# JackShDr/InfluentialRS

Measured on AMD Instinct MI355X. Metric: scored user-item pairs/sec (whole node), higher is better.
Workload: dtype f32; 1 GPU; c2: n_item=3415, d=128, L=200, H=4, layers=6, ffn=256; one greedy path-search step; users_per_gpu=4096, top_k=100, sweep=bf16 filter + exact f32 re-score, parallelism=single GPU

## Files before the change

### influentialrs_amd/csrc/capi.hip

```cpp
#include <stdlib.h>

#include <new>

#include "irs_internal.h"

int irs_launch_topk_exhaustive(irs_ctx *ctx, const float *xrows, int M, int k, float *val, int64_t *ids0,
                               int32_t *status, hipStream_t s);

static char g_create_err[512] = "";

static inline size_t align_up(size_t v, size_t a) { return (v + a - 1) / a * a; }

extern "C" int irs_abi_version(void) { return IRS_ABI_VERSION; }

extern "C" const char *irs_last_error(const irs_ctx *ctx) { return ctx ? ctx->err : g_create_err; }

extern "C" int irs_create(irs_ctx **out, const irs_dims *dims, const irs_shard *shard) {
    if (!out || !dims) {
        snprintf(g_create_err, sizeof(g_create_err), "irs_create: null argument");
        return IRS_E_INVALID;
    }
    const irs_dims &D = *dims;
#define BAD(...)                                                   \
    do {                                                           \
        snprintf(g_create_err, sizeof(g_create_err), __VA_ARGS__); \
        return IRS_E_INVALID;                                      \
    } while (0)
    if (D.n_item < 1) BAD("n_item must be >= 1");
    if (D.d < 2 || D.d > 256 || (D.d & 1)) BAD("emb_dim must be even and in [2, 256] (got %d)", D.d);
    if (D.max_len < 2 || D.max_len > 256) BAD("max_len must be in [2, 256] (got %d)", D.max_len);
    if (D.n_heads < 1 || D.d % D.n_heads) BAD("n_heads must divide emb_dim");
    if (D.d / D.n_heads > 64) BAD("head dim > 64 unsupported");
    if (D.n_layers < 1 || D.n_layers > IRS_MAX_LAYERS) BAD("n_layers out of range");
    if (D.ffn_dim < 1) BAD("ffn_dim must be >= 1");
    if (D.mask_mode != IRS_MASK_IRN && D.mask_mode != IRS_MASK_CAUSAL) BAD("bad mask_mode");
    if (D.mask_mode == IRS_MASK_IRN && (D.u_dim < 1 || D.n_user < 1)) BAD("IRN mask needs user embeddings");
    if (D.max_rows < 1) BAD("max_rows must be >= 1");
    if (D.max_k < 1 || D.max_k > 1024) BAD("max_k must be in [1, 1024]");
    irs_shard sh;
    if (shard) sh = *shard;
    else {
        sh.rank = 0;
        sh.world = 1;
        sh.item_lo = 0;
        sh.item_hi = D.n_item;
    }
    if (sh.item_lo < 0 || sh.item_hi > D.n_item || sh.item_lo >= sh.item_hi) BAD("bad item shard [%lld, %lld)", (long long)sh.item_lo, (long long)sh.item_hi);
    if (sh.item_hi - sh.item_lo > 0x7FFFFFE0LL) BAD("shard too large");
    {
        int dev = 0;
        if (hipGetDevice(&dev) == hipSuccess && (dev < 0 || dev >= IRS_MAX_DEVICES))
            BAD("device ordinal %d: contexts are supported on devices 0 .. %d", dev, IRS_MAX_DEVICES - 1);
    }
#undef BAD
    irs_ctx *c = new (std::nothrow) irs_ctx();
    if (!c) {
        snprintf(g_create_err, sizeof(g_create_err), "out of host memory");
        return IRS_E_INVALID;
    }
    memset(c, 0, sizeof(*c));
    c->dims = D;
    c->shard = sh;
    c->n_local = sh.item_hi - sh.item_lo;
    int dp = 16;
    while (dp < D.d) dp <<= 1;
    c->d_pad = dp;
    c->KS = dp / 16;
    c->n_tiles = (int)((c->n_local + 31) / 32);
    c->max_rows = D.max_rows;
    c->max_seqs = D.max_seqs > 0 ? D.max_seqs : D.max_rows;
    c->m_pad_max = (c->max_rows + 31) & ~31;
    c->lse_slots = 2048;
    {
        const char *e = getenv("IRS_DECODER_GEMM");
        if (e && strcmp(e, "f32") && strcmp(e, "x6") && strcmp(e, "h3")) {
            snprintf(g_create_err, sizeof(g_create_err), "IRS_DECODER_GEMM=%s (expected h3, x6 or f32)", e);
            delete c;
            return IRS_E_INVALID;
        }
        c->use_x6 = e ? (strcmp(e, "f32") == 0 ? IRS_GEMM_F32 : strcmp(e, "x6") == 0 ? IRS_GEMM_X6 : IRS_GEMM_H3) : IRS_GEMM_H3;
        const char *ea = getenv("IRS_ATTN_GEMM");
        if (ea && strcmp(ea, "f32") && strcmp(ea, "h3")) {
            snprintf(g_create_err, sizeof(g_create_err), "IRS_ATTN_GEMM=%s (expected h3 or f32)", ea);
            delete c;
            return IRS_E_INVALID;
        }
        c->use_attn_h3 = ea ? (strcmp(ea, "h3") == 0) : 1;
        const char *es = getenv("IRS_DECODER_SEQ");
        c->use_seq = es ? (strcmp(es, "auto") == 0 ? 2 : (atoi(es) != 0 ? 1 : 0)) : 2;
        const char *ec = getenv("IRS_THR_CARRY");
        c->carry_period = ec ? atoi(ec) : 8;
        if (c->carry_period < 0 || c->carry_period > 1024) c->carry_period = 8;
        const char *eo = getenv("IRS_SHARDED_OVERLAP");
        c->sh_overlap = eo ? (atoi(eo) != 0 ? 1 : 0) : 0;
        const char *er = getenv("IRS_LSE_RING");
        c->lse_no_ring = er ? (strcmp(er, "0") == 0) : 0;
    }
    *out = c;
    return IRS_OK;
}

extern "C" void irs_destroy(irs_ctx *ctx) {
    if (!ctx) return;
    if (ctx->graph_exec) hipGraphExecDestroy(ctx->graph_exec);
    if (ctx->beam_graph) hipGraphExecDestroy(ctx->beam_graph);
    if (ctx->sh_graph) hipGraphExecDestroy(ctx->sh_graph);
    if (ctx->sh_side) {
        for (int i = 0; i < 8; ++i) (void)hipEventDestroy(ctx->sh_ev[i]);
        (void)hipStreamDestroy(ctx->sh_side);
    }
    if (ctx->prof_ev) {
        for (int i = 0; i < ctx->prof_cap; ++i) {
            hipEventDestroy(ctx->prof_ev[i].a);
            hipEventDestroy(ctx->prof_ev[i].b);
        }
        free(ctx->prof_ev);
    }
    delete ctx;
}

static bool ends_with(const char *s, const char *suf) {
    size_t ls = strlen(s), lf = strlen(suf);
    return ls >= lf && strcmp(s + ls - lf, suf) == 0;
}

extern "C" int irs_bind_weight(irs_ctx *ctx, const char *name, const float *p, int64_t numel) {
    if (!ctx || !name || !p) return IRS_E_INVALID;
    if (strncmp(name, "module.", 7) == 0) name += 7;
    const irs_dims &D = ctx->dims;
    const int64_t d = D.d, F = D.ffn_dim;
    const float **slot = nullptr;
    int64_t want = -1;
    if (!strcmp(name, "item_embedder.weight") || !strcmp(name, "word_embedder.weight")) {
        slot = &ctx->item_emb;
        want = (D.n_item + 1) * d;
    } else if (!strcmp(name, "user_embedder.weight")) {
        slot = &ctx->user_emb;
        want = D.n_user * D.u_dim;
    } else if (!strcmp(name, "pos_embedder.pe")) {
        slot = &ctx->pe;
        want = -2;
        if (numel < (int64_t)D.max_len * d) IRS_FAIL(ctx, IRS_E_INVALID, "pos_embedder.pe too small");
    } else if (!strcmp(name, "user_mask_layer.weight")) {
        slot = &ctx->um_w;
        want = D.u_dim;
    } else if (!strcmp(name, "user_mask_layer.bias")) {
        slot = &ctx->um_b;
        want = 1;
    } else if (!strcmp(name, "project.weight")) {
        slot = &ctx->proj_w;
        want = ctx->n_local * d;
    } else if (!strcmp(name, "project.bias")) {
        slot = &ctx->proj_b;
        want = ctx->n_local;
    } else if (!strncmp(name, "decoder.layers.", 15)) {
        char *end = nullptr;
        long l = strtol(name + 15, &end, 10);
        if (l < 0 || l >= D.n_layers || !end || *end != '.') IRS_FAIL(ctx, IRS_E_INVALID, "bad layer in '%s'", name);
        const char *rest = end + 1;
        irs_layer_w &w = ctx->layer[l];
        struct { const char *n; const float **s; int64_t numel; } tab[] = {
            {"self_attn.in_proj_weight", &w.sa_in_w, 3 * d * d}, {"self_attn.in_proj_bias", &w.sa_in_b, 3 * d},
            {"self_attn.out_proj.weight", &w.sa_out_w, d * d},   {"self_attn.out_proj.bias", &w.sa_out_b, d},
            {"multihead_attn.in_proj_weight", &w.ca_in_w, 3 * d * d}, {"multihead_attn.in_proj_bias", &w.ca_in_b, 3 * d},
            {"multihead_attn.out_proj.weight", &w.ca_out_w, d * d},   {"multihead_attn.out_proj.bias", &w.ca_out_b, d},
            {"linear1.weight", &w.l1_w, F * d}, {"linear1.bias", &w.l1_b, F},
            {"linear2.weight", &w.l2_w, d * F}, {"linear2.bias", &w.l2_b, d},
            {"norm1.weight", &w.n1_w, d}, {"norm1.bias", &w.n1_b, d},
            {"norm2.weight", &w.n2_w, d}, {"norm2.bias", &w.n2_b, d},
            {"norm3.weight", &w.n3_w, d}, {"norm3.bias", &w.n3_b, d},
        };
        for (auto &e : tab)
            if (!strcmp(rest, e.n)) {
                slot = e.s;
                want = e.numel;
            }
    }
    if (!slot) IRS_FAIL(ctx, IRS_E_INVALID, "unknown weight '%s'", name);
    if (want >= 0 && numel != want) IRS_FAIL(ctx, IRS_E_INVALID, "weight '%s': numel %lld, expected %lld", name, (long long)numel, (long long)want);
    *slot = p;
    ctx->finalized = false;
    (void)ends_with;
    return IRS_OK;
}

static int check_bound(irs_ctx *ctx) {
    const irs_dims &D = ctx->dims;
    if (!ctx->item_emb || !ctx->pe || !ctx->proj_w || !ctx->proj_b) IRS_FAIL(ctx, IRS_E_STATE, "embedding / pe / project weights not bound");
    if (D.mask_mode == IRS_MASK_IRN && (!ctx->user_emb || !ctx->um_w || !ctx->um_b)) IRS_FAIL(ctx, IRS_E_STATE, "user weights not bound");
    for (int l = 0; l < D.n_layers; ++l) {
        const irs_layer_w &w = ctx->layer[l];
        const float *all[] = {w.sa_in_w, w.sa_in_b, w.sa_out_w, w.sa_out_b, w.ca_in_b, w.ca_out_w, w.ca_out_b, w.l1_w,
                              w.l1_b, w.l2_w, w.l2_b, w.n1_w, w.n1_b, w.n2_w, w.n2_b, w.n3_w, w.n3_b};
        for (auto p : all)
            if (!p) IRS_FAIL(ctx, IRS_E_STATE, "decoder layer %d has unbound weights", l);
    }
    return IRS_OK;
}

static size_t derived_plan(const irs_ctx *ctx, size_t *o_wp, size_t *o_bias, size_t *o_cl, size_t *o_wn, size_t *o_wf, size_t *o_x6 = nullptr) {
    size_t off = 0;
    *o_wp = off;
    off = align_up(off + (size_t)ctx->n_tiles * ctx->KS * 1024, 256);
    *o_bias = off;
    off = align_up(off + (size_t)ctx->n_tiles * 32 * sizeof(float), 256);
    *o_cl = off;
    off = align_up(off + (size_t)ctx->dims.n_layers * ctx->dims.d * sizeof(float), 256);
    *o_wn = off;
    off = align_up(off + 256, 256);
    *o_wf = off;
    off = align_up(off + irs_small_frag_floats(ctx) * sizeof(float), 256);
    if (o_x6) *o_x6 = off;
    off = align_up(off + irs_x6_bytes(ctx), 256);
    return off;
}

extern "C" size_t irs_derived_bytes(const irs_ctx *ctx) {
    size_t a, b, c, d, e;
    return ctx ? derived_plan(ctx, &a, &b, &c, &d, &e) : 0;
}

extern "C" int irs_finalize_weights(irs_ctx *ctx, void *arena, size_t bytes, void *stream) {
    if (!ctx || !arena) return IRS_E_INVALID;
    int rc = check_bound(ctx);
    if (rc) return rc;
    size_t o_wp, o_bias, o_cl, o_wn, o_wf, o_x6;
    size_t need = derived_plan(ctx, &o_wp, &o_bias, &o_cl, &o_wn, &o_wf, &o_x6);
    if (bytes < need) IRS_FAIL(ctx, IRS_E_INVALID, "derived arena too small: %zu < %zu", bytes, need);
    if (((uintptr_t)arena) & 255) IRS_FAIL(ctx, IRS_E_INVALID, "derived arena must be 256-byte aligned");
    char *base = (char *)arena;
    ctx->wp = (uint4 *)(base + o_wp);
    ctx->bias_pad = (float *)(base + o_bias);
    ctx->c_l = (float *)(base + o_cl);
    ctx->wnorm_max = (float *)(base + o_wn);
    ctx->w_frag16 = irs_small_frag_floats(ctx) ? (float *)(base + o_wf) : nullptr;
    ctx->w_x6 = irs_x6_bytes(ctx) ? (uint4 *)(base + o_x6) : nullptr;
    hipStream_t s = (hipStream_t)stream;
    if ((rc = irs_launch_pack_w(ctx, s))) return rc;
    if ((rc = irs_launch_cross_const(ctx, s))) return rc;
    if ((rc = irs_launch_pack_small(ctx, s))) return rc;
    if ((rc = irs_launch_pack_x6(ctx, s))) return rc;
    ctx->h3_ok = true, ctx->h3_bound = 0.f;
// ... 682 lines not shown
```

### influentialrs_amd/csrc/decoder.hip

```cpp
#include "irs_internal.h"

typedef __attribute__((ext_vector_type(16))) float f32x16;

__global__ void __launch_bounds__(256) k_embed(const int64_t *__restrict__ seq, const float *__restrict__ E,
                                               const float *__restrict__ pe, float *__restrict__ x, int rows, int L,
                                               int d, float sqrtd, int64_t n_item) {
    int row = blockIdx.x * 4 + (threadIdx.x >> 6);
    int lane = threadIdx.x & 63;
    if (row >= rows) return;
    int64_t id = seq[row];
    if (id < 0) id = 0;
    if (id > n_item) id = n_item;
    int t = row % L;
    const float *e = E + id * (int64_t)d;
    const float *p = pe + (int64_t)t * d;
    float *o = x + (int64_t)row * d;
    for (int c = lane; c < d; c += 64) o[c] = __fadd_rn(__fmul_rn(e[c], sqrtd), p[c]);
}

__global__ void k_pif(const int64_t *__restrict__ user, const float *__restrict__ U, const float *__restrict__ w,
                      const float *__restrict__ b, float *__restrict__ r_u, int B, int ud, int64_t n_user) {
    int i = blockIdx.x * blockDim.x + threadIdx.x;
    if (i >= B) return;
    int64_t u = user[i];
    if (u < 0) u = 0;
    if (u >= n_user) u = n_user - 1;
    const float *e = U + u * (int64_t)ud;
    float acc = 0.f;
    for (int c = 0; c < ud; ++c) acc = __fmaf_rn(e[c], w[c], acc);
    r_u[i] = acc + b[0];
}

__global__ void k_fill(float *p, float v, int n) {
    int i = blockIdx.x * blockDim.x + threadIdx.x;
    if (i < n) p[i] = v;
}

__global__ void k_cross_const(const float *__restrict__ Wo, const float *__restrict__ b_in, const float *__restrict__ bo,
                              float *__restrict__ c, int d) {
    int i = blockIdx.x * blockDim.x + threadIdx.x;
    if (i >= d) return;
    const float *bv = b_in + 2 * d;
    float acc = 0.f;
    for (int j = 0; j < d; ++j) acc = __fmaf_rn(Wo[(int64_t)i * d + j], bv[j], acc);
    c[i] = acc + bo[i];
}

__device__ __forceinline__ bool plan_valid(const int64_t *__restrict__ sq, int t, int L, int p) {
    return t < L && (sq[t] != 0 || t == p);
}

__global__ void __launch_bounds__(256) k_plan_count(const int64_t *__restrict__ seq, const int32_t *__restrict__ pos, int B,
                                                    int L, int32_t *__restrict__ cnt, int32_t *__restrict__ tile_seq) {
    const int b = blockIdx.x * 4 + (threadIdx.x >> 6), lane = threadIdx.x & 63;
    if (b >= B) return;
    if (tile_seq && lane < 16) tile_seq[16 * b + lane] = -1;
    int p = pos[b];
    p = p < 0 ? 0 : (p >= L ? L - 1 : p);
    const int64_t *sq = seq + (int64_t)b * L;
    int n = 0;
    for (int t0 = 0; t0 < L; t0 += 64) n += __popcll(__ballot(plan_valid(sq, t0 + lane, L, p)));
    if (lane == 0) cnt[b] = n;
}

__global__ void __launch_bounds__(1024) k_plan_scan(const int32_t *__restrict__ cnt, int B, int32_t *__restrict__ off,
                                                    int32_t *__restrict__ m_dev) {
    __shared__ int s_scan[1024];
    __shared__ int s_base;
    const int tid = threadIdx.x;
    if (tid == 0) s_base = 0;
    __syncthreads();
    for (int b0 = 0; b0 < B; b0 += 1024) {
        const int b = b0 + tid;
        const int n = (b < B) ? cnt[b] : 0;
        s_scan[tid] = n;
        __syncthreads();
        for (int o = 1; o < 1024; o <<= 1) {
            int v = (tid >= o) ? s_scan[tid - o] : 0;
            __syncthreads();
            s_scan[tid] += v;
            __syncthreads();
        }
        const int base = s_base;
        if (b < B) off[b] = base + s_scan[tid] - n;
        __syncthreads();
        if (tid == 1023) s_base = base + s_scan[1023];
        __syncthreads();
    }
    if (tid == 0) m_dev[0] = s_base;
}

__global__ void __launch_bounds__(256) k_plan_fill(const int64_t *__restrict__ seq, const int32_t *__restrict__ pos, int B,
                                                   int L, const int32_t *__restrict__ off, int32_t *__restrict__ qrow,
                                                   int32_t *__restrict__ tok_row, int32_t *__restrict__ padq) {
    const int b = blockIdx.x * 4 + (threadIdx.x >> 6), lane = threadIdx.x & 63;
    if (b >= B) return;
    int p = pos[b];
    p = p < 0 ? 0 : (p >= L ? L - 1 : p);
    const int64_t *sq = seq + (int64_t)b * L;
    int o = off[b];
    for (int t0 = 0; t0 < L; t0 += 64) {
        const int t = t0 + lane;
        const bool v = plan_valid(sq, t, L, p);
        const unsigned long long m = __ballot(v);
        if (v) {
            const int idx = o + __popcll(m & ((1ull << lane) - 1ull));
            tok_row[idx] = b * L + t;
            if (t == p) {
                qrow[b] = idx;
                padq[b] = (sq[t] == 0) ? idx - off[b] : -1;
            }
        }
        o += __popcll(m);
    }
}

static int irs_cu_count() {
    static int n_cu = 0;
    if (n_cu == 0) {
        int dev = 0;
        if (hipGetDevice(&dev) != hipSuccess ||
            hipDeviceGetAttribute(&n_cu, hipDeviceAttributeMultiprocessorCount, dev) != hipSuccess || n_cu <= 0)
            n_cu = 256;
    }
    return n_cu;
}

#define SEQ_WG_TILES 8
#define SEQ_WG_BLOCKS 16
#define SEQ_AUTO_MIN_SEQS 384
#define SEQ_RMAX 48
#define SEQ_TAIL_BLOCKS 8
#ifndef SEQ_LAB_PLAN
#define SEQ_LAB_PLAN 0
#endif
__host__ __device__ __forceinline__ int seq_half_of_block(bool slot_odd, int nb, int blk) {
    const int mir = nb - 1 - blk;
    if (!slot_odd) {
        if ((nb & 1) && blk == mir) return nb - 1;
        return blk < mir ? 2 * blk : 2 * mir + 1;
    }
    if (nb & 1) {
        if (blk == mir) return 0;
        return blk < mir ? 1 + 2 * blk : 2 + 2 * mir;
    }
    if (blk == nb / 2 - 1) return 0;
    if (blk == nb / 2) return nb - 1;
    return blk < mir ? 1 + 2 * blk : 2 + 2 * mir;
}
#define SEQ_PLAN_PER_THREAD 8
__global__ void __launch_bounds__(1024) k_plan_seq(const int32_t *__restrict__ cnt, const int32_t *__restrict__ off,
                                                   const int32_t *__restrict__ qrow, int B, int32_t *__restrict__ tile_seq,
                                                   int32_t *__restrict__ tile_qb, int32_t *__restrict__ seq_row0,
                                                   int32_t *__restrict__ qrow_tile, int32_t *__restrict__ n_wg, int tiles_cap,
                                                   int n_cu) {
    constexpr int C = SEQ_WG_BLOCKS, PT = SEQ_PLAN_PER_THREAD, CT = SEQ_TAIL_BLOCKS;
    __shared__ int s_hist[C + 1], s_start[C + 2];
    __shared__ int p_n[C], p_s[C][SEQ_RMAX], p_l[C][SEQ_RMAX];
    __shared__ int c_cum[C + 1], c_q[C], c_exist, c_newbase, s_nwg;
    __shared__ int s_cap, s_tail0, c_norm, c_nnorm;
    __shared__ unsigned short s_order[1024 * PT], s_pt[1024 * PT];
    const int tid = threadIdx.x;
    if (tid <= C) s_hist[tid] = 0;
    if (tid < C) p_n[tid] = 0;
    if (tid == 0) s_nwg = 0, s_tail0 = -1;
    __syncthreads();
    int my_T[PT], my_rk[PT];
#pragma unroll
    for (int j = 0; j < PT; ++j) {
        const int b = tid + 1024 * j;
        my_T[j] = 0, my_rk[j] = 0;
        if (b < B) {
            int nb = (cnt[b] + 15) >> 4;
            nb = nb < 1 ? 1 : (nb > C ? C : nb);
            my_T[j] = nb;
            int pt = qrow[b] - off[b];
            s_pt[b] = (unsigned short)(pt < 0 ? 0 : (pt > 65535 ? 65535 : pt));
        }
    }
#pragma unroll
    for (int j = 0; j < PT; ++j)
        if (my_T[j]) my_rk[j] = atomicAdd(&s_hist[my_T[j]], 1);
    __syncthreads();
    if (tid == 0) {
        int run = 0;
        for (int T = C; T >= 1; --T) {
            s_start[T] = run;
            run += s_hist[T];
        }
        auto count = [&](const int cap, int &nwg, int &nbig, int &ntail) __attribute__((always_inline)) {
            int dc[C];
            nwg = 0, nbig = 0, ntail = 0;
#pragma unroll
            for (int f = 0; f < C; ++f) dc[f] = 0;
#pragma unroll
            for (int T = C; T >= 1; --T) {
                int left = s_hist[T];
                if (left > 0) {
#pragma unroll
                    for (int f = T; f < C; ++f) {
                        const int q = f / T, have = dc[f] * q, used = left < have ? left : have;
                        if (used > 0) {
                            const int fl = used / q, pa = used - fl * q;
                            left -= used;
                            dc[f] -= fl + (pa ? 1 : 0), dc[f - T * q] += fl;
#pragma unroll
                            for (int p = 1; p < q; ++p)
                                if (pa == p) dc[f - T * p] += 1;
                        }
                    }
                    const int q = C / T;
                    if (T <= CT) {
                        const int qt = T <= CT ? CT / T : 1, room = cap > nwg ? cap - nwg : 0;
                        if ((long long)room * q < left) {
                            const int tl = left - room * q, flt = tl / qt, pat = tl - flt * qt;
                            left = room * q;
                            dc[CT - T * qt] += flt, nwg += flt + (pat ? 1 : 0), ntail += flt + (pat ? 1 : 0);
#pragma unroll
                            for (int p = 1; p < qt; ++p)
                                if (pat == p) dc[CT - T * p] += 1;
                        }
                    }
                    const int fl = left / q, pa = left - fl * q;
                    dc[C - T * q] += fl, nwg += fl + (pa ? 1 : 0);
#pragma unroll
                    for (int p = 1; p < q; ++p)
                        if (pa == p) dc[C - T * p] += 1;
                }
                if (T == CT + 1) nbig = nwg;
            }
        };
        int nwg, nbig, ntail;
        count(0x7FFFFFFF, nwg, nbig, ntail);
        const int rounds = n_cu > 0 ? nwg / n_cu : 0, rem = nwg - rounds * n_cu;
        s_cap = 0x7FFFFFFF;
        if (SEQ_LAB_PLAN == 0 && n_cu > 0 && rem > 0 && 2 * rem <= n_cu && nbig <= rounds * n_cu) {
            int nwg2, nbig2;
            count(rounds * n_cu, nwg2, nbig2, ntail);
            if (ntail <= n_cu) s_cap = rounds * n_cu;
        }
        if (SEQ_LAB_PLAN == 1) s_cap = 0;
        if (SEQ_LAB_PLAN == 2) s_cap = 0x7FFFFFFF;
    }
    __syncthreads();
#pragma unroll
    for (int j = 0; j < PT; ++j)
        if (my_T[j]) s_order[s_start[my_T[j]] + my_rk[j]] = (unsigned short)(tid + 1024 * j);
    __syncthreads();
    auto pool_bins = [&](int f) {
        int n = 0;
        for (int r = 0; r < p_n[f]; ++r) n += p_l[f][r];
        return n;
    };
    auto append = [&](int f, int start, int len) {
        if (f < 1 || len < 1) return;
        if (p_n[f] > 0 && p_s[f][p_n[f] - 1] + p_l[f][p_n[f] - 1] == start) p_l[f][p_n[f] - 1] += len;
        else if (p_n[f] < SEQ_RMAX) p_s[f][p_n[f]] = start, p_l[f][p_n[f]] = len, ++p_n[f];
    };
    auto take_prefix = [&](int f, int m, int dest) {
        for (int r = 0; r < p_n[f] && m > 0; ++r) {
            const int t = m < p_l[f][r] ? m : p_l[f][r];
            append(dest, p_s[f][r], t);
            p_s[f][r] += t, p_l[f][r] -= t, m -= t;
        }
        int w = 0;
        for (int r = 0; r < p_n[f]; ++r)
            if (p_l[f][r] > 0) p_s[f][w] = p_s[f][r], p_l[f][w] = p_l[f][r], ++w;
        p_n[f] = w;
    };
    for (int T = C; T >= 1; --T) {
        const int n = s_hist[T], qnew = C / T;
        if (n == 0) continue;
        if (tid == 0) {
            int tot = 0;
            for (int f = T; f < C; ++f) {
                c_cum[f] = tot, c_q[f] = f / T;
                tot += pool_bins(f) * c_q[f];
            }
            c_cum[C] = tot;
            c_exist = n < tot ? n : tot;
            c_newbase = s_nwg;
            const int nnew = n - c_exist, room = s_cap > s_nwg ? s_cap - s_nwg : 0;
            const bool spill = T <= CT && nnew > 0 && (long long)room * qnew < nnew;
            c_norm = spill ? room * qnew : nnew;
            c_nnorm = (c_norm + qnew - 1) / qnew;
            const int ntail = spill ? (nnew - c_norm + CT / T - 1) / (CT / T) : 0;
            if (ntail > 0 && s_tail0 < 0) s_tail0 = c_newbase + c_nnorm;
            s_nwg += c_nnorm + ntail;
        }
        __syncthreads();
        const int exist = c_exist, base = s_start[T];
        for (int i = tid; i < n; i += 1024) {
            const int b = s_order[base + i];
            int w, slot;
            if (i < exist) {
                int f = T;
                while (f < C - 1 && i >= c_cum[f + 1]) ++f;
                const int s_ = i - c_cum[f];
                int bl = s_ / c_q[f];
                const int k = s_ % c_q[f];
                int r = 0;
                while (r < p_n[f] - 1 && bl >= p_l[f][r]) bl -= p_l[f][r], ++r;
                w = p_s[f][r] + bl;
                slot = (C - f) + k * T;
            } else if (i - exist < c_norm) {
                const int j_ = i - exist;
                w = c_newbase + j_ / qnew;
                slot = (j_ % qnew) * T;
            } else {
                const int j_ = i - exist - c_norm, qt = CT / T;
                w = c_newbase + c_nnorm + j_ / qt;
                slot = (C - CT) + (j_ % qt) * T;
            }
            if (w * SEQ_WG_TILES >= tiles_cap) continue;
            const int h0 = 2 * SEQ_WG_TILES * w + slot;
            for (int blk = 0; blk < T; ++blk) {
                const int h = h0 + seq_half_of_block(slot & 1, T, blk);
                tile_seq[h] = b, tile_qb[h] = blk;
            }
            seq_row0[b] = 16 * slot;
            const int pt = s_pt[b];
            int pb = pt >> 4;
            pb = pb < 0 ? 0 : (pb >= T ? T - 1 : pb);
            qrow_tile[b] = 16 * (h0 + seq_half_of_block(slot & 1, T, pb)) + (pt & 15);
        }
        __syncthreads();
        if (tid == 0) {
            int left = exist;
            for (int f = T; f < C && left > 0; ++f) {
                const int q = c_q[f], cap = pool_bins(f) * q;
                const int used = left < cap ? left : cap;
                left -= used;
                const int full = used / q, part = used % q;
                take_prefix(f, full, f - T * q);
                if (part) take_prefix(f, 1, f - T * part);
            }
            const int nnew = c_norm, fullnew = nnew / qnew, partnew = nnew % qnew;
            append(C - T * qnew, c_newbase, fullnew);
            if (partnew) append(C - T * partnew, c_newbase + fullnew, 1);
            if (n - exist > c_norm) {
                const int ntl = n - exist - c_norm, qt = CT / T, fullt = ntl / qt, partt = ntl % qt;
                append(CT - T * qt, c_newbase + c_nnorm, fullt);
                if (partt) append(CT - T * partt, c_newbase + c_nnorm + fullt, 1);
            }
        }
        __syncthreads();
    }
    if (tid == 0) n_wg[0] = s_nwg, n_wg[1] = s_tail0 < 0 ? s_nwg : s_tail0;
}

__global__ void __launch_bounds__(1024) k_plan_small(const int64_t *__restrict__ seq, const int32_t *__restrict__ pos, int B, int L,
                                                     int32_t *__restrict__ cnt, int32_t *__restrict__ off,
                                                     int32_t *__restrict__ qrow, int32_t *__restrict__ tok_row,
                                                     int32_t *__restrict__ padq, int32_t *__restrict__ m_dev,
                                                     const int64_t *__restrict__ user, const float *__restrict__ U,
                                                     const float *__restrict__ uw, const float *__restrict__ ub,
                                                     float *__restrict__ r_u, int ud, int64_t n_user,
                                                     int32_t *__restrict__ step_pair) {
    __shared__ int s_cnt[64], s_off[64];
    const int tid = threadIdx.x, wave = tid >> 6, lane = tid & 63;
    for (int b = wave; b < B; b += 16) {
        int p = pos[b];
        p = p < 0 ? 0 : (p >= L ? L - 1 : p);
        const int64_t *sq = seq + (int64_t)b * L;
        int n = 0;
        for (int t0 = 0; t0 < L; t0 += 64) n += __popcll(__ballot(plan_valid(sq, t0 + lane, L, p)));
        if (lane == 0) s_cnt[b] = n;
    }
    if (tid < B) {
        float acc = 0.f;
        if (U) {
            int64_t u = user[tid];
            if (u < 0) u = 0;
            if (u >= n_user) u = n_user - 1;
            const float *e = U + u * (int64_t)ud;
            for (int c = 0; c < ud; ++c) acc = __fmaf_rn(e[c], uw[c], acc);
            acc += ub[0];
        }
        r_u[tid] = acc;
    }
    __syncthreads();
    if (tid == 0) {
        int run = 0;
        for (int b = 0; b < B; ++b) {
            s_off[b] = run;
            run += s_cnt[b];
        }
        m_dev[0] = run;
        if (step_pair) step_pair[0] = step_pair[1];
    }
    __syncthreads();
    for (int b = wave; b < B; b += 16) {
        int p = pos[b];
        p = p < 0 ? 0 : (p >= L ? L - 1 : p);
        const int64_t *sq = seq + (int64_t)b * L;
        int o = s_off[b];
        if (lane == 0) {
            cnt[b] = s_cnt[b];
            off[b] = o;
        }
        const int o0 = o;
        for (int t0 = 0; t0 < L; t0 += 64) {
            const int t = t0 + lane;
            const bool v = plan_valid(sq, t, L, p);
            const unsigned long long m = __ballot(v);
            if (v) {
                const int idx = o + __popcll(m & ((1ull << lane) - 1ull));
                tok_row[idx] = b * L + t;
                if (t == p) {
                    qrow[b] = idx;
                    padq[b] = (sq[t] == 0) ? idx - o0 : -1;
                }
            }
            o += __popcll(m);
        }
    }
}

__global__ void __launch_bounds__(256) k_embed_packed(const int64_t *__restrict__ seq, const float *__restrict__ E,
                                                      const float *__restrict__ pe, float *__restrict__ x,
                                                      const int32_t *__restrict__ tok_row, const int32_t *__restrict__ m_dev,
                                                      int L, int d, float sqrtd, int64_t n_item) {
    const int row = blockIdx.x * 4 + (threadIdx.x >> 6);
    const int lane = threadIdx.x & 63;
    if (row >= m_dev[0]) return;
    const int orig = tok_row[row];
    int64_t id = seq[orig];
    if (id < 0) id = 0;
    if (id > n_item) id = n_item;
    const float *e = E + id * (int64_t)d;
    const float *p = pe + (int64_t)(orig % L) * d;
    float *o = x + (int64_t)row * d;
    for (int c = lane; c < d; c += 64) o[c] = __fadd_rn(__fmul_rn(e[c], sqrtd), p[c]);
}

__global__ void k_gather_rows_idx(const float *__restrict__ x, const int32_t *__restrict__ rowidx, float *__restrict__ out,
                                  int d) {
    const float *src = x + (int64_t)rowidx[blockIdx.x] * d;
    for (int c = threadIdx.x; c < d; c += blockDim.x) out[(int64_t)blockIdx.x * d + c] = src[c];
}

__global__ void __launch_bounds__(256) k_embed_frag(const int64_t *__restrict__ seq, const float *__restrict__ E,
                                                    const float *__restrict__ pe, float *__restrict__ xf,
                                                    const int32_t *__restrict__ tok_row, const int32_t *__restrict__ m_dev,
                                                    int rows, int L, int d, float sqrtd, int64_t n_item) {
    const int tile = blockIdx.x * 4 + (threadIdx.x >> 6);
    const int lane = threadIdx.x & 63, li = lane & 31, lk = lane >> 5;
    const int M = m_dev ? min(rows, m_dev[0]) : rows;
    if (tile * 32 >= M) return;
    const int row = tile * 32 + li;
    const bool live = row < M;
    const int orig = live ? (tok_row ? tok_row[row] : row) : 0;
    int64_t id = live ? seq[orig] : 0;
    if (id < 0) id = 0;
    if (id > n_item) id = n_item;
    const float *e = E + id * (int64_t)d;
    const float *p = pe + (int64_t)(orig % L) * d;
    float4 *o = reinterpret_cast<float4 *>(xf) + (size_t)tile * 16 * 64 + lane;
#pragma unroll 4
    for (int c = 0; c < 16; ++c) {
        const int n = (c >> 2) * 32 + (c & 3) * 8 + 4 * lk;
        float4 v = make_float4(0.f, 0.f, 0.f, 0.f);
        if (live && n < d) {
            v.x = __fadd_rn(__fmul_rn(e[n + 0], sqrtd), p[n + 0]);
            v.y = __fadd_rn(__fmul_rn(e[n + 1], sqrtd), p[n + 1]);
            v.z = __fadd_rn(__fmul_rn(e[n + 2], sqrtd), p[n + 2]);
            v.w = __fadd_rn(__fmul_rn(e[n + 3], sqrtd), p[n + 3]);
        }
        o[c * 64] = v;
    }
}

__global__ void k_gather_rows_frag(const float *__restrict__ xf, const int32_t *__restrict__ rowidx,
                                   float *__restrict__ out, int d, int nt) {
    const int row = rowidx[blockIdx.x];
    for (int c = threadIdx.x; c < d; c += blockDim.x)
        out[(int64_t)blockIdx.x * d + c] =
            xf[(((size_t)(row >> 5) * nt + (c >> 5)) * 4 + ((c >> 3) & 3)) * 256 + ((c >> 2) & 1) * 128 + (row & 31) * 4 + (c & 3)];
}

#define LIN_BM 128
// ... 5165 lines not shown
    const irs_layer_w &w = ctx->layer[l];
    const float *cl = ctx->c_l + (size_t)l * d;
    const int32_t *m_dev = c.m_dev;
    float *xf = ctx->act_xf, *yf = ctx->act_yf;
    const hipStream_t s = c.s;
    int rc;
    const bool last = l + 1 == nl;
    const bool tail = !last && r.layer != DecFam::FRAG_GEMM;
    const bool kv_only = tail && r.kv_only && l + 2 == nl;
    BlockArgs ba{};
    ba.W1 = w.l1_w, ba.b1 = w.l1_b, ba.W2 = w.l2_w, ba.b2 = w.l2_b, ba.g = w.n3_w, ba.b = w.n3_b;
    ba.Xf = last ? nullptr : xf, ba.Y = last ? c.x : nullptr, ba.M = rows, ba.m_dev = m_dev;
    ba.Win = tail ? ctx->layer[l + 1].sa_in_w : nullptr, ba.bin = tail ? ctx->layer[l + 1].sa_in_b : nullptr;
    ba.QKV = ctx->act_qkv;
    ba.qkv_n0 = kv_only ? 128 : 0, ba.qkv_nt1 = kv_only ? 2 : 6;
    const double ffn_flops = 4.0 * rows * (double)d * F + (tail ? (kv_only ? 4.0 : 6.0) * rows * (double)d * d : 0.0);
    if (r.layer == DecFam::FRAG_FUSED) {
        ba.Af = yf, ba.Rf = xf, ba.Wo = w.sa_out_w, ba.bo = w.sa_out_b;
        ba.g1 = w.n1_w, ba.b1n = w.n1_b, ba.c = cl, ba.g2 = w.n2_w, ba.b2n = w.n2_b;
        irs_prof_begin(ctx, IRS_PROF_LINEAR, s);
        if (tail) irs_prof_begin(ctx, IRS_PROF_LAYER, s);
        if (tail && r.x6) {
            BlockX6Args xa{yf, xf, x6_stream(ctx, r.npl, l), w.sa_out_b, w.n1_w, w.n1_b, cl, w.n2_w, w.n2_b,
                           w.l1_b, w.l2_b, w.n3_w, w.n3_b, ctx->layer[l + 1].sa_in_b, xf, ctx->act_qkv, rows, m_dev, kv_only ? 1 : 0};
            xa.kv_planes = r.kv_planes ? 1 : 0;
            x6_launch(kv_only ? 1 : 0, false, r.nt, r.npl, rows, xa, s);
        } else if (r.nt == 8) IRS_FAIL(ctx, IRS_E_STATE, "d = 256 fused layer kernel without a successor layer");
        else hipLaunchKernelGGL((tail ? k_block<true, true> : k_block<true, false>), dim3((rows + 127) / 128), dim3(256), 0, s, ba);
        irs_prof_end(ctx, IRS_PROF_LINEAR, s, ffn_flops + 2.0 * rows * (double)d * d, (8.0 + 4.0 + (tail ? 12.0 : 0.0)) * rows * (double)d);
        if (tail) irs_prof_end(ctx, IRS_PROF_LAYER, s, ffn_flops + 2.0 * rows * (double)d * d, (8.0 + 4.0 + 12.0) * rows * (double)d);
        return IRS_OK;
    }
    if ((rc = launch_linear(ctx, ctx->act_ao, w.sa_out_w, w.sa_out_b, nullptr, nullptr, rows, d, d, false, s, w.n1_w, w.n1_b, cl,
                            w.n2_w, w.n2_b, xf, yf, m_dev)))
        return rc;
    if (r.layer == DecFam::FRAG_BLOCK) {
        ba.Yf = yf;
        irs_prof_begin(ctx, IRS_PROF_LINEAR, s);
        hipLaunchKernelGGL((tail ? k_block<false, true> : k_block<false, false>), dim3((rows + 127) / 128), dim3(256), 0, s, ba);
        irs_prof_end(ctx, IRS_PROF_LINEAR, s, ffn_flops, (8.0 + (tail ? 12.0 : 0.0)) * rows * (double)d);
        return IRS_OK;
    }
    if ((rc = launch_linear(ctx, nullptr, w.l1_w, w.l1_b, nullptr, ctx->act_h, rows, F, d, true, s, nullptr, nullptr, nullptr, nullptr,
                            nullptr, nullptr, nullptr, m_dev, yf)))
        return rc;
    return launch_linear(ctx, ctx->act_h, w.l2_w, w.l2_b, nullptr, last ? c.x : nullptr, rows, d, F, false, s, w.n3_w, w.n3_b, nullptr,
                         nullptr, nullptr, yf, last ? nullptr : xf, m_dev);
}

static int decode_layer(DecodeCall &c, int l) {
    irs_ctx *ctx = c.ctx;
    const DecodeRoute &r = c.r;
    float *x = c.x, *y = c.y;
    int rc;
    const bool fused = r.layer == DecFam::FRAG_FUSED;
    if (!r.att_fused && (rc = launch_attn(ctx, ctx->act_qkv, c.seq, ctx->act_ru, fused ? ctx->act_yf : ctx->act_ao, c.B, c.s, c.off,
                                          c.cnt, c.tok, fused, r.kv_planes)))
        return rc;
    switch (r.layer) {
    case DecFam::FRAG_GEMM:
    case DecFam::FRAG_BLOCK:
    case DecFam::FRAG_FUSED:
        return frag_layer(c, l);
    case DecFam::SMALL16:
    case DecFam::WIDE:
    case DecFam::ANY: {
        SmallBlockArgs sb = small_args(ctx, r.layer, l, ctx->act_ao, x, nullptr, y, qkv_buf(c, l + 1), c.rows, c.m_dev,
                                       l + 1 < ctx->dims.n_layers);
        if (r.att_fused) {
            sb.QKVin = qkv_buf(c, l), sb.r_u = ctx->act_ru, sb.seq_last = c.seq + (ctx->dims.max_len - 1), sb.cnt = c.cnt;
            sb.padq = ctx->seq_padq, sb.mask_mode = ctx->dims.mask_mode;
        }
        launch_small(ctx, r.layer, sb, r.att_fused, c.rows > SMALL_MT2_ROWS, c.s);
        c.x = y;
        c.y = x;
        return IRS_OK;
    }
    default:
        return gemm_rest(ctx, r.layer == DecFam::GEMM_LN, l, ctx->act_ao, x, r.layer == DecFam::GEMM_LN ? y : x, y, x, c.rows, c.m_dev,
                         c.s);
    }
}

static int last_layer(const DecodeCall &c, int l, const int32_t *pos, float *xrows) {
    irs_ctx *ctx = c.ctx;
    const DecodeRoute &r = c.r;
    const int L = ctx->dims.max_len, d = ctx->dims.d, H = ctx->dims.n_heads, B = c.B;
    const irs_layer_w &w = ctx->layer[l];
    const int32_t *qrow = c.qrow;
    const hipStream_t s = c.s;
    int rc;
    float *xf = ctx->act_xf, *h_r = ctx->act_h;
    float *ao_r = ctx->act_ao, *x_r = ao_r + (size_t)B * d, *y_r = ao_r + (size_t)2 * B * d, *z_r = ao_r + (size_t)3 * B * d;
    const float *q_r = nullptr;
    const int nt = d > 128 ? d / 32 : 4;
    if (r.seq) {
        hipLaunchKernelGGL(k_gather_rows_frag, dim3(B), dim3(64), 0, s, xf, ctx->qrow_tile, x_r, d, nt);
        hipLaunchKernelGGL(k_gather_rows_frag, dim3(B), dim3(64), 0, s, ctx->act_yf, ctx->qrow_tile, ao_r, d, nt);
    } else if (r.kv_only) {
        hipLaunchKernelGGL(k_gather_rows_frag, dim3(B), dim3(64), 0, s, xf, qrow, x_r, d, nt);
        if ((rc = launch_linear(ctx, x_r, w.sa_in_w, w.sa_in_b, nullptr, h_r, B, d, d, false, s))) return rc;
        q_r = h_r;
    }
    irs_prof_begin(ctx, IRS_PROF_ATTN, s);
    if (r.seq) {
    } else if (d / H == 32 && L <= 256 && d % 4 == 0 && (((uintptr_t)ctx->act_qkv | (uintptr_t)q_r) & 15) == 0)
        hipLaunchKernelGGL(k_attn_row32, dim3(H, B), dim3(256), 0, s, ctx->act_qkv, c.seq, ctx->act_ru, ao_r, L, d,
                           ctx->dims.mask_mode, c.off, c.cnt, qrow, q_r, ctx->seq_padq);
    else
        hipLaunchKernelGGL(k_attn_row, dim3(H, B), dim3(64), 0, s, ctx->act_qkv, c.seq, ctx->act_ru, pos, ao_r, L, d, d / H,
                           ctx->dims.mask_mode, c.off, c.cnt, c.tok, qrow, q_r);
    irs_prof_end(ctx, IRS_PROF_ATTN, s, 4.0 * B * (double)L * d, 4.0 * 3.0 * B * (double)L * d);
    const bool small = r.tail == DecFam::SMALL16 || r.tail == DecFam::WIDE || r.tail == DecFam::ANY;
    const bool idx_res = small && !r.frag;
    if (r.frag && !r.kv_only) hipLaunchKernelGGL(k_gather_rows_frag, dim3(B), dim3(64), 0, s, xf, qrow, x_r, d, nt);
    else if (!r.frag && !idx_res) hipLaunchKernelGGL(k_gather_rows_idx, dim3(B), dim3(64), 0, s, c.x, qrow, x_r, d);
    if (small) {
        const SmallBlockArgs sb = small_args(ctx, r.tail, l, ao_r, idx_res ? c.x : x_r, idx_res ? qrow : nullptr, xrows, nullptr, B,
                                             nullptr, false);
        launch_small(ctx, r.tail, sb, false, B > 2048, s);
    } else if ((rc = gemm_rest(ctx, r.tail == DecFam::GEMM_LN, l, ao_r, x_r, y_r, z_r, xrows, B, nullptr, s))) {
        return rc;
    }
    IRS_CHECK_HIP(ctx, hipGetLastError());
    return IRS_OK;
}

int irs_launch_decode(irs_ctx *ctx, const int64_t *seq, const int64_t *user, int B, float *x_out, const int32_t *pos,
                      float *xrows, float *r_u_out, hipStream_t s) {
    const int L = ctx->dims.max_len, d = ctx->dims.d, nl = ctx->dims.n_layers;
    const DecodeRoute r = decode_route(ctx, B, x_out == nullptr && pos && xrows && L >= 4);
    int rc;
    if (ctx->step_pair && !r.small_plan) IRS_FAIL(ctx, IRS_E_STATE, "merged path step needs the single-workgroup plan kernel");
    if (!r.small_plan && (rc = irs_launch_pif(ctx, user, B, ctx->act_ru, s)) != IRS_OK) return rc;
    ctx->seq_last = r.seq;
    const int32_t packed[IRS_ROUTE_FIELDS] = {r.rows_only, r.small_plan, (int32_t)r.plan, (int32_t)r.embed, (int32_t)r.layer,
                                              (int32_t)r.tail, r.frag, r.seq, r.kv_planes, r.att_fused, r.kv_only, r.x6, r.npl, r.nt};
    for (int i = 0; i < IRS_ROUTE_FIELDS; ++i) ctx->route_last[i] = packed[i];
    ctx->route_n = IRS_ROUTE_FIELDS;
    DecodeCall c{ctx, r, seq, B, B * L, ctx->act_x, ctx->act_y, s};
    if (r.rows_only) c.off = ctx->seq_off, c.cnt = ctx->seq_cnt, c.tok = ctx->tok_row, c.qrow = ctx->seq_qrow, c.m_dev = ctx->m_dev;
    if (r.plan == DecPlan::SMALL) {
        hipLaunchKernelGGL(k_plan_small, dim3(1), dim3(1024), 0, s, seq, pos, B, L, ctx->seq_cnt, ctx->seq_off, ctx->seq_qrow,
                           ctx->tok_row, ctx->seq_padq, ctx->m_dev, user, pif_table(ctx), ctx->um_w, ctx->um_b, ctx->act_ru,
                           ctx->dims.u_dim, ctx->dims.n_user, ctx->step_pair);
    } else if (r.plan == DecPlan::MULTI) {
        hipLaunchKernelGGL(k_plan_count, dim3((B + 3) / 4), dim3(256), 0, s, seq, pos, B, L, ctx->seq_cnt, ctx->tile_seq);
        hipLaunchKernelGGL(k_plan_scan, dim3(1), dim3(1024), 0, s, ctx->seq_cnt, B, ctx->seq_off, ctx->m_dev);
        hipLaunchKernelGGL(k_plan_fill, dim3((B + 3) / 4), dim3(256), 0, s, seq, pos, B, L, ctx->seq_off, ctx->seq_qrow, ctx->tok_row,
                           ctx->seq_padq);
    }
    const int n_cu = r.seq ? irs_cu_count() : 0;
    if (r.seq)
        hipLaunchKernelGGL(k_plan_seq, dim3(1), dim3(1024), 0, s, ctx->seq_cnt, ctx->seq_off, ctx->seq_qrow, B, ctx->tile_seq,
                           ctx->tile_idx, ctx->seq_row0, ctx->qrow_tile, ctx->n_wg_dev, B * SEQ_WG_TILES, n_cu);
    launch_embed(c, pos, user);
    IRS_CHECK_HIP(ctx, hipGetLastError());
    if (r_u_out) IRS_CHECK_HIP(ctx, hipMemcpyAsync(r_u_out, ctx->act_ru, sizeof(float) * B, hipMemcpyDeviceToDevice, s));
    const bool embed_qkv = r.embed == DecEmbed::SEQ || r.embed == DecEmbed::FRAG_QKV || r.embed == DecEmbed::SMALL16_QKV ||
                           r.embed == DecEmbed::ANY_QKV;
    const int l0 = r.seq ? nl - 1 : 0;
    for (int l = l0; l < nl; ++l) {
        const irs_layer_w &w = ctx->layer[l];
        if (!(l == l0 ? embed_qkv : fam_writes_qkv(r.layer)) &&
            (rc = launch_linear(ctx, c.x, w.sa_in_w, w.sa_in_b, nullptr, ctx->act_qkv, c.rows, 3 * d, d, false, s, nullptr, nullptr,
                                nullptr, nullptr, nullptr, nullptr, nullptr, c.m_dev, r.frag ? ctx->act_xf : nullptr)))
            return rc;
        if (r.rows_only && l + 1 == nl) return last_layer(c, l, pos, xrows);
        if ((rc = decode_layer(c, l))) return rc;
        IRS_CHECK_HIP(ctx, hipGetLastError());
    }
    if (x_out) IRS_CHECK_HIP(ctx, hipMemcpyAsync(x_out, c.x, sizeof(float) * (size_t)c.rows * d, hipMemcpyDeviceToDevice, s));
    if (pos && xrows) {
        hipLaunchKernelGGL(k_gather_rows, dim3(B), dim3(64), 0, s, c.x, pos, xrows, B, L, d);
        IRS_CHECK_HIP(ctx, hipGetLastError());
    }
    return IRS_OK;
}
```

### influentialrs_amd/csrc/irs_internal.h

```cpp
#pragma once

#include <hip/hip_runtime.h>
#include <stdint.h>
#include <stdio.h>
#include <string.h>

#include "../../include/irs_hip.h"

#if !defined(IRS_LAB) && (defined(X6_DUMP) || defined(X6_STAMP) || defined(X6_NO_SPLIT) || defined(X6_STAGGER) ||            \
                          defined(X6_NO_MFMA) || defined(X6_NO_READS) || defined(X6_NO_DMA) || defined(X6_NO_BARRIER) ||       \
                          defined(X6_NW) || defined(ATTN_STAMP) || defined(ATTNP_STAMP) ||               \
                          defined(IRS_SMALL_TIMING) || defined(IRS_DIRECT_TIMING) || defined(SWEEP_LAB) || defined(X6D_STAMP) ||              \
                          defined(X6_NO_QKV_STORE) || defined(X6_NSLOT2) || defined(X6_RESID_LATE) || defined(X6_RING4) ||      \
                          defined(X6_SPLIT_ACC4) || defined(SEQ_EXP))
#error "a lab switch (X6_* / ATTN* / IRS_*_TIMING) is defined without IRS_LAB: the product library must be built without them"
#endif

#include <atomic>
#define IRS_MAX_DEVICES 32
static inline int irs_cur_dev() {
    int d = 0;
    if (hipGetDevice(&d) != hipSuccess || d < 0 || d >= IRS_MAX_DEVICES) d = 0;
    return d;
}
#define IRS_ONCE_PER_DEVICE(body_)                                                                                        \
    do {                                                                                                                  \
        static std::atomic<unsigned> once_mask_{0};                                                                       \
        const unsigned once_bit_ = 1u << irs_cur_dev();                                                                   \
        if (!(once_mask_.load(std::memory_order_acquire) & once_bit_)) {                                                  \
            body_;                                                                                                        \
            once_mask_.fetch_or(once_bit_, std::memory_order_release);                                                    \
        }                                                                                                                 \
    } while (0)

#define IRS_MAX_LAYERS 16
#define IRS_CAND_BUCKETS 64
#define IRS_CAND_SLOTS 64
#define IRS_CAND_CAP (IRS_CAND_BUCKETS * IRS_CAND_SLOTS)
#define IRS_REFINE_CAP 1024
#define IRS_MAX_GROUPS 2048
#define IRS_MAX_PATH 64
#define IRS_LSE_SLOTS_RING 4096
#define IRS_COOP_FALLBACK_MIN_ITEMS 262144
#define IRS_EXH_SCRATCH_KEYS (64 * 32768)

struct irs_layer_w {
    const float *sa_in_w, *sa_in_b, *sa_out_w, *sa_out_b;
    const float *ca_in_w, *ca_in_b, *ca_out_w, *ca_out_b;
    const float *l1_w, *l1_b, *l2_w, *l2_b;
    const float *n1_w, *n1_b, *n2_w, *n2_b, *n3_w, *n3_b;
};

struct irs_prof_ev {
    hipEvent_t a, b;
};

struct irs_ctx {
    irs_dims dims;
    irs_shard shard;
    int64_t n_local;
    int d_pad;
    int KS;
    int n_tiles;
    int max_seqs;
    int max_rows;
    int m_pad_max;

    const float *item_emb, *user_emb, *pe, *um_w, *um_b, *proj_w, *proj_b;
    irs_layer_w layer[IRS_MAX_LAYERS];

    uint4 *wp;
    float *bias_pad;
    float *c_l;
    float *wnorm_max;
    float *w_frag16;
    uint4 *w_x6;
    int use_x6;
    bool h3_ok;
    float h3_bound;
    int use_seq;
    bool seq_last;
    int32_t route_last[IRS_ROUTE_FIELDS];
    int route_n;
    int use_attn_h3;
    int lse_no_ring;
    bool finalized;
    bool proj_stale;

    char *ws;
    size_t ws_bytes;
    float *act_x, *act_y, *act_qkv, *act_ao, *act_h, *act_ru;
    float *act_qkv_b1;
    float *act_xf, *act_yf;
    int32_t *tok_row;
    int32_t *seq_cnt, *seq_off, *seq_qrow;
    int32_t *seq_padq;
    int32_t *m_dev;
    int32_t *tile_seq, *tile_idx;
    int32_t *seq_row0, *qrow_tile;
    int32_t *n_wg_dev;
    uint4 *xb;
    float *eps;
    float *thr;
    float *gm;
    unsigned int *cand_cnt;
    unsigned long long *cand;
    float *lse_part;
    int lse_slots;
    float *ref_tmp;
    int thr_valid, thr_M, thr_k, thr_age, carry_period;
    unsigned int *fb_count;
    int32_t *fb_list;
    unsigned long long *exh_keys;
    float *xrows;
    float *top_val;
    int64_t *top_ids;
    int32_t *row_status;
    int32_t *step_ctr;
    int32_t *step_pair;
    int32_t *pos_tmp;
    int64_t *bm_seq[2];
    int32_t *bm_hep[2];
    double *bm_cum[2];
    float *bm_paths[2];
    int64_t *bm_user;
    float *lse_max, *lse_sum;
    float *x_local;
    uint64_t *keys_send, *keys_recv;
    float *lse_gmax;
    hipGraphExec_t sh_graph;
    int sh_kind, sh_B, sh_W, sh_P, sh_k, sh_sweep, sh_sample, sh_sample_k, sh_nograph;
    int sh_overlap;
    hipStream_t sh_side;
    hipEvent_t sh_ev[8];
    uint64_t sh_seed;
    void *sh_comm, *sh_ptr[5];
    hipGraphExec_t beam_graph;
    int beam_B, beam_W, beam_k, beam_sweep, beam_P;
    void *beam_status;

    hipGraphExec_t graph_exec;
    int graph_B, graph_P, graph_k, graph_sweep, graph_sample, graph_sample_k;
    void *graph_seq, *graph_user, *graph_hep, *graph_paths, *graph_status;
    uint64_t graph_seed;

    int prof_family;
    irs_prof_ev *prof_ev;
    int prof_n, prof_cap;
    double prof_flops, prof_bytes;

    char err[512];
};

#define IRS_CHECK_HIP(ctx, expr)                                                                         \
    do {                                                                                                 \
        hipError_t _e = (expr);                                                                          \
        if (_e != hipSuccess) {                                                                          \
            snprintf((ctx)->err, sizeof((ctx)->err), "%s:%d %s -> %s", __FILE__, __LINE__, #expr,        \
                     hipGetErrorString(_e));                                                             \
            return IRS_E_HIP;                                                                            \
        }                                                                                                \
    } while (0)

#define IRS_FAIL(ctx, code, ...)                                  \
    do {                                                          \
        snprintf((ctx)->err, sizeof((ctx)->err), __VA_ARGS__);    \
        return (code);                                            \
    } while (0)

void irs_prof_begin(irs_ctx *ctx, int family, hipStream_t s);
void irs_prof_end(irs_ctx *ctx, int family, hipStream_t s, double flops, double bytes);

static inline bool irs_seq_shape(const irs_dims &D) {
    return D.d == 128 && D.ffn_dim == 256 && D.n_heads == 4 && D.max_len <= 256 && D.n_layers > 1;
}
static inline bool irs_small_plan(const irs_dims &D, int B) { return B <= 64 && D.max_len >= 4; }

int irs_launch_pif(irs_ctx *ctx, const int64_t *user, int B, float *r_u, hipStream_t s);
int irs_launch_decode(irs_ctx *ctx, const int64_t *seq, const int64_t *user, int B, float *x_out, const int32_t *pos,
                      float *xrows, float *r_u_out, hipStream_t s);
int irs_launch_cross_const(irs_ctx *ctx, hipStream_t s);
size_t irs_small_frag_floats(const irs_ctx *ctx);
int irs_launch_pack_small(irs_ctx *ctx, hipStream_t s);
size_t irs_x6_bytes(const irs_ctx *ctx);
int irs_launch_pack_x6(irs_ctx *ctx, hipStream_t s);
int irs_launch_h3_range(irs_ctx *ctx, float *stats, hipStream_t s);
float irs_h3_operand_bound(const irs_ctx *ctx, const float *stats);

int irs_launch_pack_w(irs_ctx *ctx, hipStream_t s);
struct irs_path_args;
bool irs_topk_is_direct(const irs_ctx *ctx, int M, int k);
int irs_launch_topk(irs_ctx *ctx, const float *xrows, int M, int k, int sweep, float *val, int64_t *ids0,
                    int32_t *status, hipStream_t s, const irs_path_args *path = nullptr, float *lse_max = nullptr,
                    float *lse_sum = nullptr, int carry = 0);
int irs_launch_gather(irs_ctx *ctx, const float *xrows, int M, const int64_t *ids0, int g, float *out, hipStream_t s);
int irs_launch_count_before(irs_ctx *ctx, const float *xrows, int M, const float *ref_score, const int64_t *ref_id0,
                            const int64_t *excl, int n_excl, int64_t *count, hipStream_t s);
int irs_launch_dense(irs_ctx *ctx, const float *xrows, int M, float *out, int64_t ld, hipStream_t s);
int irs_launch_lse(irs_ctx *ctx, const float *xrows, int M, float *out_max, float *out_sum, hipStream_t s);
int irs_launch_refresh_bias(irs_ctx *ctx, hipStream_t s);
int irs_launch_lse_combine(irs_ctx *ctx, const float *mx, const float *sm, float *lse, int M, hipStream_t s);
int irs_launch_ce_reduce(irs_ctx *ctx, const float *lse, const float *lab_score, const int64_t *labels0, int M, double *out,
                         hipStream_t s);
int irs_launch_ce_grad(irs_ctx *ctx, const float *xrows, const int64_t *labels0, const float *lse, int M, float scale,
                       float *out, int64_t ld, hipStream_t s);

int irs_launch_merge(irs_ctx *ctx, const float *val_in, const int64_t *ids_in, int W, int M, int k, float *val,
                     int64_t *ids0, hipStream_t s);
int irs_launch_merge_keys(irs_ctx *ctx, const uint64_t *keys_in, int W, int M, int k, float *val, int64_t *ids0, hipStream_t s);
int irs_launch_pack_topk(irs_ctx *ctx, const float *val, const int64_t *ids0, int64_t n, uint64_t *keys, hipStream_t s);
int irs_launch_path_step(irs_ctx *ctx, int64_t *seq, int32_t *hep, int B, const float *val, const int64_t *ids0, int k,
                         int step, const int32_t *step_ptr, float *paths, int path_ld, int sample, int sample_k,
                         uint64_t seed, int32_t *status, hipStream_t s, int32_t *step_next = nullptr);
int irs_launch_inc(irs_ctx *ctx, int32_t *ctr, hipStream_t s);
int irs_launch_beam_init(irs_ctx *ctx, const int64_t *seq0, const int64_t *user0, const int32_t *hep0, int B, int W,
                         int P, int64_t *seq, int64_t *user, int32_t *hep, double *cum, float *paths, hipStream_t s);
int irs_launch_beam_step(irs_ctx *ctx, const int64_t *seq_in, const int32_t *hep_in, const double *cum_in,
                         const float *paths_in, const float *val, const int64_t *ids0, const float *lse_max,
                         const float *lse_sum, int B, int W, int k, int step, const int32_t *step_ptr, int P,
                         int64_t *seq_out, int32_t *hep_out, double *cum_out, float *paths_out, int32_t *status,
                         hipStream_t s);

int irs_launch_build_eval_batch(irs_ctx *ctx, const int64_t *items, const int64_t *offsets, int B, int raw_len, int gap_len,
                                const int64_t *targets_in, const int64_t *pool, int64_t n_pool, uint64_t seed, int64_t *seq,
                                int64_t *target, int64_t *label, int64_t *raw, int32_t *raw_n, int32_t *status,
                                hipStream_t s);

#ifdef __HIPCC__
__device__ __forceinline__ unsigned int irs_fkey(float f) {
    unsigned int u = __float_as_uint(f);
    if (u == 0x80000000u) u = 0u;
    return (u & 0x80000000u) ? ~u : (u | 0x80000000u);
}
__device__ __forceinline__ float irs_unkey(unsigned int k) {
// ... 170 lines not shown
```

Measured before the change: 2.203 billion pairs/s.

## Parallelize sequence tile planning across a wavefront instead of one thread

```diff
diff --git a/influentialrs_amd/csrc/capi.hip b/influentialrs_amd/csrc/capi.hip
--- a/influentialrs_amd/csrc/capi.hip
+++ b/influentialrs_amd/csrc/capi.hip
@@ -88,6 +88,13 @@
         c->use_attn_h3 = ea ? (strcmp(ea, "h3") == 0) : 1;
         const char *es = getenv("IRS_DECODER_SEQ");
         c->use_seq = es ? (strcmp(es, "auto") == 0 ? 2 : (atoi(es) != 0 ? 1 : 0)) : 2;
+        const char *ep = getenv("IRS_SEQ_PLAN");
+        if (ep && strcmp(ep, "parallel") && strcmp(ep, "serial")) {
+            snprintf(g_create_err, sizeof(g_create_err), "IRS_SEQ_PLAN=%s (expected parallel or serial)", ep);
+            delete c;
+            return IRS_E_INVALID;
+        }
+        c->seq_plan_serial = ep ? (strcmp(ep, "serial") == 0) : 0;
         const char *ec = getenv("IRS_THR_CARRY");
         c->carry_period = ec ? atoi(ec) : 8;
         if (c->carry_period < 0 || c->carry_period > 1024) c->carry_period = 8;
diff --git a/influentialrs_amd/csrc/decoder.hip b/influentialrs_amd/csrc/decoder.hip
--- a/influentialrs_amd/csrc/decoder.hip
+++ b/influentialrs_amd/csrc/decoder.hip
@@ -149,6 +149,66 @@
     return blk < mir ? 1 + 2 * blk : 2 + 2 * mir;
 }
 #define SEQ_PLAN_PER_THREAD 8
+#define SEQ_WAVE_SYNC() do { __builtin_amdgcn_fence(__ATOMIC_SEQ_CST, "wavefront"); __builtin_amdgcn_wave_barrier(); } while (0)
+__device__ __forceinline__ int plan_scan16(int v, int lane, int &tot) {
+    int incl = v;
+#pragma unroll
+    for (int o = 1; o < 16; o <<= 1) {
+        const int u = __shfl_up(incl, o, 16);
+        if ((lane & 15) >= o) incl += u;
+    }
+    tot = __shfl(incl, 15);
+    return incl - v;
+}
+__device__ __forceinline__ void plan_count_wave(const int *hist, int *dc, const int lane, const int cap, int &nwg, int &nbig,
+                                                int &ntail) {
+    constexpr int C = SEQ_WG_BLOCKS, CT = SEQ_TAIL_BLOCKS;
+    if (lane < C) dc[lane] = 0;
+    SEQ_WAVE_SYNC();
+    nwg = 0, nbig = 0, ntail = 0;
+    for (int T = C; T >= 1; --T) {
+        int left = hist[T];
+        if (left > 0) {
+            const bool act = lane >= T && lane < C;
+            const int qf = act ? lane / T : 1, have = act ? dc[lane] * qf : 0;
+            int tot;
+            const int cum = plan_scan16(have, lane, tot);
+            int used = left - cum;
+            used = used < 0 ? 0 : (used > have ? have : used);
+            SEQ_WAVE_SYNC();
+            if (used > 0) {
+                const int fl = used / qf, pa = used - fl * qf;
+                atomicAdd(&dc[lane], -(fl + (pa ? 1 : 0)));
+                if (fl) atomicAdd(&dc[lane - T * qf], fl);
+                if (pa) atomicAdd(&dc[lane - T * pa], 1);
+            }
+            SEQ_WAVE_SYNC();
+            left -= left < tot ? left : tot;
+            const int q = C / T;
+            if (T <= CT) {
+                const int qt = CT / T, room = cap > nwg ? cap - nwg : 0;
+                if ((long long)room * q < left) {
+                    const int tl = left - room * q, flt = tl / qt, pat = tl - flt * qt;
+                    left = room * q;
+                    nwg += flt + (pat ? 1 : 0), ntail += flt + (pat ? 1 : 0);
+                    if (lane == 0) {
+                        dc[CT - T * qt] += flt;
+                        if (pat) dc[CT - T * pat] += 1;
+                    }
+                }
+            }
+            const int fl = left / q, pa = left - fl * q;
+            nwg += fl + (pa ? 1 : 0);
+            if (lane == 0) {
+                dc[C - T * q] += fl;
+                if (pa) dc[C - T * pa] += 1;
+            }
+            SEQ_WAVE_SYNC();
+        }
+        if (T == CT + 1) nbig = nwg;
+    }
+}
+template <bool PAR>
 __global__ void __launch_bounds__(1024) k_plan_seq(const int32_t *__restrict__ cnt, const int32_t *__restrict__ off,
                                                    const int32_t *__restrict__ qrow, int B, int32_t *__restrict__ tile_seq,
                                                    int32_t *__restrict__ tile_qb, int32_t *__restrict__ seq_row0,
@@ -160,6 +220,7 @@
     __shared__ int c_cum[C + 1], c_q[C], c_exist, c_newbase, s_nwg;
     __shared__ int s_cap, s_tail0, c_norm, c_nnorm;
     __shared__ unsigned short s_order[1024 * PT], s_pt[1024 * PT];
+    __shared__ int s_dc[C], m_n[C], m_s[C][SEQ_RMAX], m_l[C][SEQ_RMAX];
     const int tid = threadIdx.x;
     if (tid <= C) s_hist[tid] = 0;
     if (tid < C) p_n[tid] = 0;
@@ -182,7 +243,26 @@
     for (int j = 0; j < PT; ++j)
         if (my_T[j]) my_rk[j] = atomicAdd(&s_hist[my_T[j]], 1);
     __syncthreads();
-    if (tid == 0) {
+    if (PAR && tid < 64) {
+        if (tid >= 1 && tid <= C) {
+            int run = 0;
+            for (int T = C; T > tid; --T) run += s_hist[T];
+            s_start[tid] = run;
+        }
+        int nwg, nbig, ntail;
+        plan_count_wave(s_hist, s_dc, tid, 0x7FFFFFFF, nwg, nbig, ntail);
+        const int rounds = n_cu > 0 ? nwg / n_cu : 0, rem = nwg - rounds * n_cu;
+        int cap = 0x7FFFFFFF;
+        if (SEQ_LAB_PLAN == 0 && n_cu > 0 && rem > 0 && 2 * rem <= n_cu && nbig <= rounds * n_cu) {
+            int nwg2, nbig2;
+            plan_count_wave(s_hist, s_dc, tid, rounds * n_cu, nwg2, nbig2, ntail);
+            if (ntail <= n_cu) cap = rounds * n_cu;
+        }
+        if (SEQ_LAB_PLAN == 1) cap = 0;
+        if (SEQ_LAB_PLAN == 2) cap = 0x7FFFFFFF;
+        if (tid == 0) s_cap = cap;
+    }
+    if (!PAR && tid == 0) {
         int run = 0;
         for (int T = C; T >= 1; --T) {
             s_start[T] = run;
@@ -271,12 +351,21 @@
     for (int T = C; T >= 1; --T) {
         const int n = s_hist[T], qnew = C / T;
         if (n == 0) continue;
+        int l_q = 1, l_have = 0, l_cum = 0;
+        int tot = 0;
+        if (PAR && tid < 64) {
+            const bool act = tid >= T && tid < C;
+            l_q = act ? tid / T : 1;
+            l_have = act ? pool_bins(tid) * l_q : 0;
+            l_cum = plan_scan16(l_have, tid, tot);
+            if (act) c_cum[tid] = l_cum, c_q[tid] = l_q;
+        }
         if (tid == 0) {
-            int tot = 0;
-            for (int f = T; f < C; ++f) {
-                c_cum[f] = tot, c_q[f] = f / T;
-                tot += pool_bins(f) * c_q[f];
-            }
+            if (!PAR)
+                for (int f = T; f < C; ++f) {
+                    c_cum[f] = tot, c_q[f] = f / T;
+                    tot += pool_bins(f) * c_q[f];
+                }
             c_cum[C] = tot;
             c_exist = n < tot ? n : tot;
             c_newbase = s_nwg;
@@ -312,7 +401,7 @@
                 w = c_newbase + c_nnorm + j_ / qt;
                 slot = (C - CT) + (j_ % qt) * T;
             }
-            if (w * SEQ_WG_TILES >= tiles_cap) continue;
+            if (w < 0 || w * SEQ_WG_TILES >= tiles_cap) continue;
             const int h0 = 2 * SEQ_WG_TILES * w + slot;
             for (int blk = 0; blk < T; ++blk) {
                 const int h = h0 + seq_half_of_block(slot & 1, T, blk);
@@ -325,8 +414,46 @@
             qrow_tile[b] = 16 * (h0 + seq_half_of_block(slot & 1, T, pb)) + (pt & 15);
         }
         __syncthreads();
+        if (PAR && tid < 64) {
+            const int f = tid;
+            int used = exist - l_cum;
+            used = used < 0 ? 0 : (used > l_have ? l_have : used);
+            const int full = used / l_q, part = used - full * l_q;
+            if (f < C) m_n[f] = 0;
+            if (full + (part ? 1 : 0) > 0) {
+                int m = full + (part ? 1 : 0), w = 0, ns = 0;
+                const int pn = p_n[f];
+                for (int r = 0; r < pn; ++r) {
+                    int st = p_s[f][r], ln = p_l[f][r];
+                    const int t = m < ln ? m : ln;
+                    if (t > 0) m_s[f][ns] = st, m_l[f][ns] = t, ++ns, st += t, ln -= t, m -= t;
+                    if (ln > 0) p_s[f][w] = st, p_l[f][w] = ln, ++w;
+                }
+                p_n[f] = w, m_n[f] = ns;
+            }
+            SEQ_WAVE_SYNC();
+            for (int g = T; g < C; ++g) {
+                const int gf = __shfl(full, g), gp = __shfl(part, g);
+                if (gf == 0 && gp == 0) continue;
+                const int d1 = g - T * (g / T), d2 = g - T * gp;
+                if (f == d1 && gf > 0) {
+                    int m = gf;
+                    for (int r = 0; r < m_n[g] && m > 0; ++r) {
+                        const int t = m < m_l[g][r] ? m : m_l[g][r];
+                        append(d1, m_s[g][r], t);
+                        m -= t;
+                    }
+                }
+                if (f == d2 && gp > 0) {
+                    int m = gf, r = 0;
+                    while (r < m_n[g] - 1 && m >= m_l[g][r]) m -= m_l[g][r], ++r;
+                    append(d2, m_s[g][r] + m, 1);
+                }
+            }
+            SEQ_WAVE_SYNC();
+        }
         if (tid == 0) {
-            int left = exist;
+            int left = PAR ? 0 : exist;
             for (int f = T; f < C && left > 0; ++f) {
                 const int q = c_q[f], cap = pool_bins(f) * q;
                 const int used = left < cap ? left : cap;
@@ -5798,7 +5925,7 @@
     }
     const int n_cu = r.seq ? irs_cu_count() : 0;
     if (r.seq)
-        hipLaunchKernelGGL(k_plan_seq, dim3(1), dim3(1024), 0, s, ctx->seq_cnt, ctx->seq_off, ctx->seq_qrow, B, ctx->tile_seq,
+        hipLaunchKernelGGL(ctx->seq_plan_serial ? k_plan_seq<false> : k_plan_seq<true>, dim3(1), dim3(1024), 0, s, ctx->seq_cnt, ctx->seq_off, ctx->seq_qrow, B, ctx->tile_seq,
                            ctx->tile_idx, ctx->seq_row0, ctx->qrow_tile, ctx->n_wg_dev, B * SEQ_WG_TILES, n_cu);
     launch_embed(c, pos, user);
     IRS_CHECK_HIP(ctx, hipGetLastError());
diff --git a/influentialrs_amd/csrc/irs_internal.h b/influentialrs_amd/csrc/irs_internal.h
--- a/influentialrs_amd/csrc/irs_internal.h
+++ b/influentialrs_amd/csrc/irs_internal.h
@@ -80,6 +80,7 @@
     float h3_bound;
     int use_seq;
     bool seq_last;
+    int seq_plan_serial;
     int32_t route_last[IRS_ROUTE_FIELDS];
     int route_n;
     int use_attn_h3;
```

Result: no change. 2.191 billion pairs/s (-0.5%).
